# onesamblack/distributed-torch-horovod-gcp

Hardware: NVIDIA H100
Metric: images/sec (whole job, device-timed, max over ranks) ResNet-50 synthetic ImageNet training (higher is better)
Workload: dtype bf16

## Files before the change

### distributed_torch_horovod_gcp_b200/csrc/elementwise.cu

```cuda
#include <cuda_bf16.h>
#include <cuda_runtime.h>
#include <stdint.h>
#include <stdio.h>

namespace {

constexpr int THREADS = 256;

__device__ __forceinline__ void unpack8(const uint4& x, float* f) {
  const uint32_t w[4] = {x.x, x.y, x.z, x.w};
#pragma unroll
  for (int t = 0; t < 4; ++t) {
    f[2 * t] = __uint_as_float(w[t] << 16);
    f[2 * t + 1] = __uint_as_float(w[t] & 0xffff0000u);
  }
}
__device__ __forceinline__ uint4 pack8(const float* v) {
  uint32_t w[4];
#pragma unroll
  for (int t = 0; t < 4; ++t) {
    __nv_bfloat162 h = __floats2bfloat162_rn(v[2 * t], v[2 * t + 1]);
    w[t] = *reinterpret_cast<uint32_t*>(&h);
  }
  return make_uint4(w[0], w[1], w[2], w[3]);
}
__device__ __forceinline__ uint4 ldg_stream(const uint4* p) {
  uint4 v;
  asm volatile("ld.global.nc.L1::no_allocate.v4.u32 {%0,%1,%2,%3}, [%4];"
               : "=r"(v.x), "=r"(v.y), "=r"(v.z), "=r"(v.w)
               : "l"(p));
  return v;
}

constexpr int RED_MAX_BLOCKS = 256;
constexpr int RED_MAX_COLS = 2 * 2048;
__device__ float g_red_slots[RED_MAX_BLOCKS * RED_MAX_COLS];
__device__ unsigned int g_red_done;

template <int NACC, int NT>
__device__ __forceinline__ void block_reduce_to_global(float (&acc)[NACC][8], int V, float* const* outs) {
  __shared__ float sm[NT][8 + 1];
  __shared__ bool last;
  const int tid = threadIdx.x;
  const int groups = NT / V;
  const int C = V * 8;
  float* slot = g_red_slots + (size_t)blockIdx.x * (NACC * C);
#pragma unroll
  for (int q = 0; q < NACC; ++q) {
    __syncthreads();
#pragma unroll
    for (int j = 0; j < 8; ++j) sm[tid][j] = acc[q][j];
    __syncthreads();
    for (int item = tid; item < C; item += NT) {
      const int g0 = item >> 3, j = item & 7;
      float s = 0.f;
      for (int g = 0; g < groups; ++g) s += sm[g0 + g * V][j];
      slot[q * C + item] = s;
    }
  }
  __threadfence();
  __syncthreads();
  if (tid == 0) last = atomicAdd(&g_red_done, 1u) == gridDim.x - 1;
  __syncthreads();
  if (!last) return;
  __threadfence();
  for (int item = tid; item < NACC * C; item += NT) {
    float s = 0.f;
    for (unsigned b = 0; b < gridDim.x; ++b) s += __ldcg(g_red_slots + (size_t)b * (NACC * C) + item);
    outs[item / C][item % C] += s;
  }
  if (tid == 0) g_red_done = 0u;
}

constexpr int RTHREADS = 1024;

__device__ __forceinline__ uint4 ld_or_zero(const uint4* p, long long i, long long n) {
  return i < n ? ldg_stream(p + i) : make_uint4(0, 0, 0, 0);
}

__global__ void __launch_bounds__(RTHREADS, 1) bn_stats_kernel(const uint4* __restrict__ x, float* sum,
                                                               float* sumsq, long long nvec, int V) {
  constexpr int U = 8;
  float acc[2][8];
#pragma unroll
  for (int j = 0; j < 8; ++j) acc[0][j] = acc[1][j] = 0.f;
  const long long stride = (long long)gridDim.x * RTHREADS;
  for (long long i = (long long)blockIdx.x * RTHREADS + threadIdx.x; i < nvec; i += U * stride) {
    uint4 raw[U];
#pragma unroll
    for (int u = 0; u < U; ++u) raw[u] = ld_or_zero(x, i + u * stride, nvec);
#pragma unroll
    for (int u = 0; u < U; ++u) {
      float f[8];
      unpack8(raw[u], f);
#pragma unroll
      for (int j = 0; j < 8; ++j) {
        acc[0][j] += f[j];
        acc[1][j] = fmaf(f[j], f[j], acc[1][j]);
      }
    }
  }
  float* outs[2] = {sum, sumsq};
  block_reduce_to_global<2, RTHREADS>(acc, V, outs);
}

__device__ __forceinline__ float ld_param(const void* p, int c, int bf16) {
  return bf16 ? __bfloat162float(reinterpret_cast<const __nv_bfloat16*>(p)[c])
              : reinterpret_cast<const float*>(p)[c];
}
__device__ __forceinline__ void st_param(void* p, int c, int bf16, float v) {
  if (bf16) reinterpret_cast<__nv_bfloat16*>(p)[c] = __float2bfloat16_rn(v);
  else reinterpret_cast<float*>(p)[c] = v;
}

__global__ void bn_finalize_kernel(float* sum, float* sumsq, const void* gamma,
                                   const void* beta, float* mean, float* invstd, float* a, float* b,
                                   void* running_mean, void* running_var, float count, float eps,
                                   float momentum, int C, int pbf16, int rezero = 0,
                                   long long* num_batches_tracked = nullptr) {
  const int c = blockIdx.x * blockDim.x + threadIdx.x;
  if (c == 0 && num_batches_tracked != nullptr) *num_batches_tracked += 1;
  if (c >= C) return;
  const float m = sum[c] / count;
  const float var = fmaxf(sumsq[c] / count - m * m, 0.f);
  if (rezero) {
    sum[c] = 0.f;
    sumsq[c] = 0.f;
  }
  const float is = rsqrtf(var + eps);
  mean[c] = m;
  invstd[c] = is;
  const float g = gamma ? ld_param(gamma, c, pbf16) : 1.f;
  a[c] = g * is;
  b[c] = (beta ? ld_param(beta, c, pbf16) : 0.f) - m * g * is;
  if (running_mean) {
    const float unbiased = var * (count / fmaxf(count - 1.f, 1.f));
    st_param(running_mean, c, pbf16, (1.f - momentum) * ld_param(running_mean, c, pbf16) + momentum * m);
    st_param(running_var, c, pbf16,
             (1.f - momentum) * ld_param(running_var, c, pbf16) + momentum * unbiased);
  }
}

__global__ void __launch_bounds__(THREADS, 4) bn_apply_kernel(const uint4* __restrict__ x,
                                                              const uint4* __restrict__ res, uint4* y,
                                                              const float* __restrict__ a,
                                                              const float* __restrict__ b, long long nvec,
                                                              int V, int relu, uint8_t* __restrict__ mask) {
  constexpr int U = 4;
  const long long stride = (long long)gridDim.x * THREADS;
  const long long i0 = (long long)blockIdx.x * THREADS + threadIdx.x;
  if (i0 >= nvec) return;
  const int cg = (int)(i0 % V);
  float av[8], bv[8];
#pragma unroll
  for (int j = 0; j < 8; ++j) {
    av[j] = a[cg * 8 + j];
    bv[j] = b[cg * 8 + j];
  }
  for (long long i = i0; i < nvec; i += U * stride) {
    uint4 rx[U], rr[U];
#pragma unroll
    for (int u = 0; u < U; ++u) rx[u] = ld_or_zero(x, i + u * stride, nvec);
    if (res) {
#pragma unroll
      for (int u = 0; u < U; ++u) rr[u] = ld_or_zero(res, i + u * stride, nvec);
    }
#pragma unroll
    for (int u = 0; u < U; ++u) {
      if (i + u * stride >= nvec) break;
      float f[8];
      unpack8(rx[u], f);
#pragma unroll
      for (int j = 0; j < 8; ++j) f[j] = fmaf(f[j], av[j], bv[j]);
      if (res) {
        float r[8];
        unpack8(rr[u], r);
#pragma unroll
        for (int j = 0; j < 8; ++j) f[j] += r[j];
      }
      if (relu) {
        if (mask) {
          uint32_t m = 0;
#pragma unroll
          for (int j = 0; j < 8; ++j) m |= (f[j] > 0.f ? 1u : 0u) << j;
          mask[i + u * stride] = (uint8_t)m;
        }
#pragma unroll
        for (int j = 0; j < 8; ++j) f[j] = fmaxf(f[j], 0.f);
      }
      y[i + u * stride] = pack8(f);
    }
  }
}

__global__ void __launch_bounds__(RTHREADS, 1) bn_bwd_reduce_kernel(
    const uint4* __restrict__ dy, const uint4* __restrict__ x, const uint8_t* __restrict__ mask,
    const float* __restrict__ mean, float* sum_dy, float* sum_dy_xc, long long nvec, int V, int relu) {
  constexpr int U = 2;
  float acc[2][8];
#pragma unroll
  for (int j = 0; j < 8; ++j) acc[0][j] = acc[1][j] = 0.f;
  const long long stride = (long long)gridDim.x * RTHREADS;
  const long long i0 = (long long)blockIdx.x * RTHREADS + threadIdx.x;
  float mv[8];
  {
    const int cg = (int)(i0 % V);
#pragma unroll
    for (int j = 0; j < 8; ++j) mv[j] = mean[cg * 8 + j];
  }
  for (long long i = i0; i < nvec; i += U * stride) {
    uint4 rg[U], rx[U];
    uint32_t rm[U];
#pragma unroll
    for (int u = 0; u < U; ++u) {
      rg[u] = ld_or_zero(dy, i + u * stride, nvec);
      rx[u] = ld_or_zero(x, i + u * stride, nvec);
      rm[u] = (relu && i + u * stride < nvec) ? (uint32_t)__ldg(mask + i + u * stride) : 0xffu;
    }
#pragma unroll
    for (int u = 0; u < U; ++u) {
      float g[8], xv[8];
      unpack8(rg[u], g);
      unpack8(rx[u], xv);
#pragma unroll
      for (int j = 0; j < 8; ++j) g[j] = ((rm[u] >> j) & 1u) ? g[j] : 0.f;
#pragma unroll
      for (int j = 0; j < 8; ++j) {
        acc[0][j] += g[j];
        acc[1][j] = fmaf(g[j], xv[j] - mv[j], acc[1][j]);
      }
    }
  }
  float* outs[2] = {sum_dy, sum_dy_xc};
  block_reduce_to_global<2, RTHREADS>(acc, V, outs);
}

__global__ void __launch_bounds__(THREADS, 4) bn_bwd_apply_kernel(
    const uint4* __restrict__ dy, const uint4* __restrict__ x, const uint8_t* __restrict__ mask, uint4* dx,
    uint4* dres, const float* __restrict__ mean, const float* __restrict__ invstd,
    const float* __restrict__ scale_a, const float* __restrict__ sum_dy,
    const float* __restrict__ sum_dy_xhat, float inv_count, long long nvec, int V, int relu,
    void* dgamma, void* dbeta, int pbf16) {
  constexpr int U = 2;
  const long long stride = (long long)gridDim.x * THREADS;
  const long long i0 = (long long)blockIdx.x * THREADS + threadIdx.x;
  if (blockIdx.x == 0 && dgamma != nullptr) {
    for (int c = threadIdx.x; c < V * 8; c += THREADS) {
      st_param(dbeta, c, pbf16, sum_dy[c]);
      st_param(dgamma, c, pbf16, sum_dy_xhat[c] * invstd[c]);
    }
  }
  if (i0 >= nvec) return;
  const int cg = (int)(i0 % V);
  float mv[8], iv[8], k1[8], k2[8], sc[8];
#pragma unroll
  for (int j = 0; j < 8; ++j) {
    const int c = cg * 8 + j;
    mv[j] = mean[c];
    iv[j] = invstd[c];
    sc[j] = scale_a[c];
    k1[j] = sum_dy[c] * inv_count;
    k2[j] = sum_dy_xhat[c] * iv[j] * inv_count;
  }
  for (long long i = i0; i < nvec; i += U * stride) {
    uint4 rg[U], rx[U];
    uint32_t rm[U];
#pragma unroll
    for (int u = 0; u < U; ++u) {
      rg[u] = ld_or_zero(dy, i + u * stride, nvec);
      rx[u] = ld_or_zero(x, i + u * stride, nvec);
      rm[u] = (relu && i + u * stride < nvec) ? (uint32_t)__ldg(mask + i + u * stride) : 0xffu;
    }
#pragma unroll
    for (int u = 0; u < U; ++u) {
      if (i + u * stride >= nvec) break;
      float g[8], xv[8], o[8];
      unpack8(rg[u], g);
      unpack8(rx[u], xv);
#pragma unroll
      for (int j = 0; j < 8; ++j) g[j] = ((rm[u] >> j) & 1u) ? g[j] : 0.f;
#pragma unroll
      for (int j = 0; j < 8; ++j) {
        const float xhat = (xv[j] - mv[j]) * iv[j];
        o[j] = sc[j] * (g[j] - k1[j] - xhat * k2[j]);
      }
      dx[i + u * stride] = pack8(o);
      if (dres) dres[i + u * stride] = pack8(g);
    }
  }
}

constexpr int LN_WARPS = 16;

template <int VPL>
__global__ void __launch_bounds__(LN_WARPS * 32) ln_fwd_kernel(const uint4* __restrict__ x, uint4* __restrict__ y,
                                                               const void* gamma, const void* beta,
                                                               float* __restrict__ mean, float* __restrict__ rstd,
                                                               long long rows, float eps, int pbf16) {
  constexpr int C = 256 * VPL;
  const int lane = threadIdx.x & 31;
  const long long warp = (long long)blockIdx.x * LN_WARPS + (threadIdx.x >> 5);
  const long long nwarps = (long long)gridDim.x * LN_WARPS;
  float g[VPL][8], b[VPL][8];
#pragma unroll
  for (int v = 0; v < VPL; ++v)
#pragma unroll
    for (int j = 0; j < 8; ++j) {
      const int c = (v * 32 + lane) * 8 + j;
      g[v][j] = ld_param(gamma, c, pbf16);
      b[v][j] = ld_param(beta, c, pbf16);
    }
  for (long long r = warp; r < rows; r += nwarps) {
    const uint4* xr = x + r * (C / 8);
    float f[VPL][8];
    float s = 0.f;
#pragma unroll
    for (int v = 0; v < VPL; ++v) {
      unpack8(ldg_stream(xr + v * 32 + lane), f[v]);
#pragma unroll
      for (int j = 0; j < 8; ++j) s += f[v][j];
    }
#pragma unroll
    for (int o = 16; o > 0; o >>= 1) s += __shfl_xor_sync(0xffffffffu, s, o);
    const float m = s * (1.f / C);
    float q = 0.f;
#pragma unroll
    for (int v = 0; v < VPL; ++v)
#pragma unroll
      for (int j = 0; j < 8; ++j) {
        const float d = f[v][j] - m;
        q = fmaf(d, d, q);
      }
#pragma unroll
    for (int o = 16; o > 0; o >>= 1) q += __shfl_xor_sync(0xffffffffu, q, o);
    const float rs = rsqrtf(q * (1.f / C) + eps);
    if (lane == 0) {
      mean[r] = m;
      rstd[r] = rs;
    }
    uint4* yr = y + r * (C / 8);
#pragma unroll
    for (int v = 0; v < VPL; ++v) {
      float o[8];
#pragma unroll
      for (int j = 0; j < 8; ++j) o[j] = fmaf((f[v][j] - m) * rs, g[v][j], b[v][j]);
      yr[v * 32 + lane] = pack8(o);
    }
  }
}

template <int VPL>
__global__ void __launch_bounds__(LN_WARPS * 32) ln_bwd_kernel(const uint4* __restrict__ dy,
                                                               const uint4* __restrict__ x, uint4* __restrict__ dx,
                                                               const void* gamma, const float* __restrict__ mean,
                                                               const float* __restrict__ rstd, float* sums,
                                                               long long rows, int pbf16) {
  constexpr int C = 256 * VPL;
  extern __shared__ float red[];
  const int lane = threadIdx.x & 31, wib = threadIdx.x >> 5;
  const long long warp = (long long)blockIdx.x * LN_WARPS + wib;
  const long long nwarps = (long long)gridDim.x * LN_WARPS;
  float g[VPL][8], dg[VPL][8], db[VPL][8];
#pragma unroll
  for (int v = 0; v < VPL; ++v)
#pragma unroll
    for (int j = 0; j < 8; ++j) {
      g[v][j] = ld_param(gamma, (v * 32 + lane) * 8 + j, pbf16);
      dg[v][j] = db[v][j] = 0.f;
    }
  for (long long r = warp; r < rows; r += nwarps) {
    const float m = mean[r], rs = rstd[r];
// ... 202 lines not shown
  }
  const int vec_per_row = row_elems / 8;
  for (int i = threadIdx.x; i < 7 * vec_per_row; i += THREADS) {
    const int r = i / vec_per_row, v = i % vec_per_row;
    const int ih = oh * 2 - 3 + r;
    uint4 val = make_uint4(0, 0, 0, 0);
    if (ih >= 0 && ih < H)
      val = reinterpret_cast<const uint4*>(x + ((size_t)n * H + ih) * row_elems)[v];
    __nv_bfloat16* d = rows + r * pitch + 9 + v * 8;
    const __nv_bfloat16* sv = reinterpret_cast<const __nv_bfloat16*>(&val);
#pragma unroll
    for (int e = 0; e < 8; ++e) d[e] = sv[e];
  }
  __syncthreads();
  constexpr int UPR = STEM_KP / 8;
  uint4* dst = out + ((size_t)n * OH + oh) * OW * UPR;
  const uint32_t* rows32 = reinterpret_cast<const uint32_t*>(rows);
  const int pitch32 = pitch / 2;
  for (int i = threadIdx.x; i < OW * UPR; i += THREADS) {
    const int ow = i / UPR, u = i % UPR;
    const int kh = u / 3, part = u % 3;
    const uint32_t* src = rows32 + kh * pitch32 + ow * 3 + part * 4;
    dst[i] = make_uint4(src[0], src[1], src[2], src[3]);
  }
}


__global__ void __launch_bounds__(THREADS) avgpool_fwd_kernel(const uint4* __restrict__ x, uint4* __restrict__ y,
                                                              int HW, int V, long long total, float inv) {
  for (long long i = (long long)blockIdx.x * THREADS + threadIdx.x; i < total; i += (long long)gridDim.x * THREADS) {
    const long long n = i / V;
    const int v = (int)(i % V);
    const uint4* src = x + n * HW * V + v;
    float acc[8];
#pragma unroll
    for (int j = 0; j < 8; ++j) acc[j] = 0.f;
    for (int h = 0; h < HW; ++h) {
      float f[8];
      unpack8(src[(long long)h * V], f);
#pragma unroll
      for (int j = 0; j < 8; ++j) acc[j] += f[j];
    }
#pragma unroll
    for (int j = 0; j < 8; ++j) acc[j] *= inv;
    y[i] = pack8(acc);
  }
}
__global__ void __launch_bounds__(THREADS) avgpool_bwd_kernel(const uint4* __restrict__ dy, uint4* __restrict__ dx,
                                                              int HW, int V, long long total, float inv) {
  for (long long i = (long long)blockIdx.x * THREADS + threadIdx.x; i < total; i += (long long)gridDim.x * THREADS) {
    const long long n = i / ((long long)HW * V);
    const int v = (int)(i % V);
    float f[8];
    unpack8(dy[n * V + v], f);
#pragma unroll
    for (int j = 0; j < 8; ++j) f[j] *= inv;
    dx[i] = pack8(f);
  }
}

thread_local char g_err[256];
int fail(const char* what, cudaError_t e) {
  snprintf(g_err, sizeof(g_err), "%s: %s", what, cudaGetErrorString(e));
  return -1;
}

int g_sms = 0;
int reduce_grid() {
  if (g_sms == 0) {
    int dev = 0;
    cudaGetDevice(&dev);
    cudaDeviceGetAttribute(&g_sms, cudaDevAttrMultiProcessorCount, dev);
    if (g_sms <= 0) g_sms = 132;
    if (g_sms > RED_MAX_BLOCKS) g_sms = RED_MAX_BLOCKS;
  }
  return g_sms;
}

int grid_for(long long nvec, int V) {
  long long blocks = (nvec + THREADS * 8 - 1) / (THREADS * 8);
  if (blocks > (long long)reduce_grid() * 6) blocks = (long long)reduce_grid() * 6;
  if (blocks < 1) blocks = 1;
  return (int)blocks;
}

template <bool OUT_BF16>
__global__ void cast_acc_zero_kernel(float* __restrict__ src, void* __restrict__ dst, long long n4,
                                     int accumulate, int zero_src) {
  const long long stride = (long long)gridDim.x * blockDim.x;
  for (long long i = (long long)blockIdx.x * blockDim.x + threadIdx.x; i < n4; i += stride) {
    float4 v = reinterpret_cast<float4*>(src)[i];
    if (zero_src) reinterpret_cast<float4*>(src)[i] = make_float4(0.f, 0.f, 0.f, 0.f);
    if (OUT_BF16) {
      uint2* d = reinterpret_cast<uint2*>(dst) + i;
      if (accumulate) {
        const uint2 o = *d;
        v.x += __uint_as_float(o.x << 16); v.y += __uint_as_float(o.x & 0xffff0000u);
        v.z += __uint_as_float(o.y << 16); v.w += __uint_as_float(o.y & 0xffff0000u);
      }
      __nv_bfloat162 lo = __floats2bfloat162_rn(v.x, v.y), hi = __floats2bfloat162_rn(v.z, v.w);
      *d = make_uint2(*reinterpret_cast<uint32_t*>(&lo), *reinterpret_cast<uint32_t*>(&hi));
    } else {
      float4* d = reinterpret_cast<float4*>(dst) + i;
      if (accumulate) { const float4 o = *d; v.x += o.x; v.y += o.y; v.z += o.z; v.w += o.w; }
      *d = v;
    }
  }
}

bool shape_ok(int C) {
  const int V = C / 8;
  return C % 8 == 0 && V >= 1 && V <= THREADS && (THREADS % V) == 0;
}

}

extern "C" {

const char* b200dp_ew_last_error() { return g_err; }

int b200dp_cast_acc_zero(void* src, void* dst, long long n, int out_bf16, int accumulate, int zero_src,
                         unsigned long long stream) {
  if (n % 4) {
    snprintf(g_err, sizeof(g_err), "cast_acc_zero: n must be a multiple of 4");
    return -1;
  }
  const long long n4 = n / 4;
  int grid = (int)((n4 + 255) / 256);
  if (grid > reduce_grid() * 8) grid = reduce_grid() * 8;
  if (grid < 1) grid = 1;
  cudaStream_t st = (cudaStream_t)(uintptr_t)stream;
  if (out_bf16) cast_acc_zero_kernel<true><<<grid, 256, 0, st>>>((float*)src, dst, n4, accumulate, zero_src);
  else cast_acc_zero_kernel<false><<<grid, 256, 0, st>>>((float*)src, dst, n4, accumulate, zero_src);
  cudaError_t e = cudaGetLastError();
  if (e != cudaSuccess) return fail("cast_acc_zero launch", e);
  return 0;
}

int b200dp_bn_supported(int C) { return shape_ok(C) ? 1 : 0; }

int b200dp_bn_fwd(const void* x, const void* res, void* y, const void* gamma, const void* beta,
                  float* stats, float* mean, float* invstd, float* a, float* b, void* running_mean,
                  void* running_var, long long M, int C, float eps, float momentum, int relu,
                  int param_bf16, int have_stats, void* relu_mask, void* num_batches_tracked,
                  unsigned long long stream) {
  if (!shape_ok(C)) {
    snprintf(g_err, sizeof(g_err), "unsupported channel count %d", C);
    return -1;
  }
  cudaStream_t st = (cudaStream_t)(uintptr_t)stream;
  const int V = C / 8;
  const long long nvec = M * V;
  cudaError_t e = cudaSuccess;
  const int grid = grid_for(nvec, V);
  if (!have_stats) {
    e = cudaMemsetAsync(stats, 0, sizeof(float) * 2 * C, st);
    if (e != cudaSuccess) return fail("memset", e);
    bn_stats_kernel<<<reduce_grid(), RTHREADS, 0, st>>>((const uint4*)x, stats, stats + C, nvec, V);
  }
  bn_finalize_kernel<<<(C + 127) / 128, 128, 0, st>>>(stats, stats + C, gamma, beta, mean, invstd, a, b,
                                                      running_mean, running_var, (float)M, eps, momentum, C,
                                                      param_bf16, have_stats == 2 ? 1 : 0,
                                                      (long long*)num_batches_tracked);
  bn_apply_kernel<<<grid, THREADS, 0, st>>>((const uint4*)x, (const uint4*)res, (uint4*)y, a, b, nvec, V,
                                            relu, (uint8_t*)relu_mask);
  e = cudaGetLastError();
  if (e != cudaSuccess) return fail("bn_fwd launch", e);
  return 0;
}

int b200dp_bn_stats(const void* x, float* stats, long long M, int C, unsigned long long stream) {
  if (!shape_ok(C)) return -1;
  cudaStream_t st = (cudaStream_t)(uintptr_t)stream;
  cudaError_t e = cudaMemsetAsync(stats, 0, sizeof(float) * 2 * C, st);
  if (e != cudaSuccess) return fail("memset", e);
  bn_stats_kernel<<<reduce_grid(), RTHREADS, 0, st>>>((const uint4*)x, stats, stats + C, (long long)M * (C / 8),
                                                      C / 8);
  e = cudaGetLastError();
  if (e != cudaSuccess) return fail("bn_stats launch", e);
  return 0;
}

int b200dp_bn_fwd_sync(const void* x, const void* res, void* y, const void* gamma, const void* beta,
                       const float* stats, float* mean, float* invstd, float* a, float* b, void* running_mean,
                       void* running_var, long long M_local, double count, int C, float eps, float momentum,
                       int relu, int param_bf16, void* relu_mask, unsigned long long stream) {
  if (!shape_ok(C)) return -1;
  cudaStream_t st = (cudaStream_t)(uintptr_t)stream;
  const int V = C / 8;
  const long long nvec = M_local * V;
  bn_finalize_kernel<<<(C + 127) / 128, 128, 0, st>>>(const_cast<float*>(stats), const_cast<float*>(stats) + C, gamma,
                                                      beta, mean, invstd, a, b, running_mean, running_var,
                                                      (float)count, eps, momentum, C, param_bf16);
  bn_apply_kernel<<<grid_for(nvec, V), THREADS, 0, st>>>((const uint4*)x, (const uint4*)res, (uint4*)y, a, b, nvec,
                                                         V, relu, (uint8_t*)relu_mask);
  cudaError_t e = cudaGetLastError();
  if (e != cudaSuccess) return fail("bn_fwd_sync launch", e);
  return 0;
}

int b200dp_bn_bwd_reduce(const void* dy, const void* x, const void* relu_mask, const float* mean, float* sums,
                         long long M, int C, int relu, unsigned long long stream) {
  if (!shape_ok(C)) return -1;
  cudaStream_t st = (cudaStream_t)(uintptr_t)stream;
  cudaError_t e = cudaMemsetAsync(sums, 0, sizeof(float) * 2 * C, st);
  if (e != cudaSuccess) return fail("memset", e);
  bn_bwd_reduce_kernel<<<reduce_grid(), RTHREADS, 0, st>>>((const uint4*)dy, (const uint4*)x,
                                                           (const uint8_t*)relu_mask, mean, sums, sums + C,
                                                           (long long)M * (C / 8), C / 8, relu);
  e = cudaGetLastError();
  if (e != cudaSuccess) return fail("bn_bwd_reduce launch", e);
  return 0;
}

int b200dp_bn_bwd_apply(const void* dy, const void* x, const void* relu_mask, void* dx, void* dres,
                        const float* scale_a, const float* mean, const float* invstd, const float* sums,
                        double count, long long M, int C, int relu, unsigned long long stream) {
  if (!shape_ok(C)) return -1;
  const int V = C / 8;
  const long long nvec = M * V;
  bn_bwd_apply_kernel<<<grid_for(nvec, V), THREADS, 0, (cudaStream_t)(uintptr_t)stream>>>(
      (const uint4*)dy, (const uint4*)x, (const uint8_t*)relu_mask, (uint4*)dx, (uint4*)dres, mean, invstd, scale_a,
      sums, sums + C, (float)(1.0 / count), nvec, V, relu, nullptr, nullptr, 0);
  cudaError_t e = cudaGetLastError();
  if (e != cudaSuccess) return fail("bn_bwd_apply launch", e);
  return 0;
}

int b200dp_bn_apply(const void* x, const void* res, void* y, const float* a, const float* b, long long M,
                    int C, int relu, unsigned long long stream) {
  if (!shape_ok(C)) return -1;
  const int V = C / 8;
  const long long nvec = M * V;
  bn_apply_kernel<<<grid_for(nvec, V), THREADS, 0, (cudaStream_t)(uintptr_t)stream>>>(
      (const uint4*)x, (const uint4*)res, (uint4*)y, a, b, nvec, V, relu, nullptr);
  cudaError_t e = cudaGetLastError();
  if (e != cudaSuccess) return fail("bn_apply launch", e);
  return 0;
}

int b200dp_bn_bwd(const void* dy, const void* x, const void* relu_mask, void* dx, void* dres, const float* scale_a,
                  const float* mean, const float* invstd, float* sums, void* dgamma, void* dbeta,
                  int param_bf16, long long M, int C, int relu, unsigned long long stream) {
  if (!shape_ok(C)) return -1;
  cudaStream_t st = (cudaStream_t)(uintptr_t)stream;
  const int V = C / 8;
  const long long nvec = M * V;
  cudaError_t e = cudaMemsetAsync(sums, 0, sizeof(float) * 2 * C, st);
  if (e != cudaSuccess) return fail("memset", e);
  const int grid = grid_for(nvec, V);
  bn_bwd_reduce_kernel<<<reduce_grid(), RTHREADS, 0, st>>>((const uint4*)dy, (const uint4*)x,
                                                           (const uint8_t*)relu_mask, mean, sums, sums + C,
                                                           nvec, V, relu);
  bn_bwd_apply_kernel<<<grid, THREADS, 0, st>>>((const uint4*)dy, (const uint4*)x, (const uint8_t*)relu_mask,
                                                (uint4*)dx, (uint4*)dres, mean, invstd, scale_a, sums,
                                                sums + C, 1.0f / (float)M, nvec, V, relu, dgamma, dbeta,
                                                param_bf16);
  e = cudaGetLastError();
  if (e != cudaSuccess) return fail("bn_bwd launch", e);
  return 0;
}

int b200dp_maxpool_fwd(const void* x, void* y, void* idx, int N, int H, int W, int C,
                       unsigned long long stream) {
  if (C % 8) return -1;
  const int OH = (H + 2 - 3) / 2 + 1, OW = (W + 2 - 3) / 2 + 1, V = C / 8;
  const long long total = (long long)N * OH * OW * V;
  int grid = (int)((total + THREADS - 1) / THREADS);
  if (grid > reduce_grid() * 16) grid = reduce_grid() * 16;
  maxpool_fwd_kernel<<<grid, THREADS, 0, (cudaStream_t)(uintptr_t)stream>>>((const uint4*)x, (uint4*)y,
                                                                             (uint2*)idx, N, H, W, OH, OW, V);
  cudaError_t e = cudaGetLastError();
  if (e != cudaSuccess) return fail("maxpool_fwd launch", e);
  return 0;
}

int b200dp_maxpool_bwd(const void* dy, const void* idx, void* dx, int N, int H, int W, int C,
                       unsigned long long stream) {
  if (C % 8) return -1;
  const int OH = (H + 2 - 3) / 2 + 1, OW = (W + 2 - 3) / 2 + 1, V = C / 8;
  if (H % 2 == 0 && W % 2 == 0) {
    const long long patches = (long long)N * (H / 2) * (W / 2) * V;
    int pgrid = (int)((patches + THREADS - 1) / THREADS);
    if (pgrid > reduce_grid() * 16) pgrid = reduce_grid() * 16;
    maxpool_bwd_patch_kernel<<<pgrid, THREADS, 0, (cudaStream_t)(uintptr_t)stream>>>(
        (const uint4*)dy, (const uint2*)idx, (uint4*)dx, N, H, W, OH, OW, V);
    cudaError_t pe = cudaGetLastError();
    if (pe != cudaSuccess) return fail("maxpool_bwd launch", pe);
    return 0;
  }
  const long long total = (long long)N * H * W * V;
  int grid = (int)((total + THREADS - 1) / THREADS);
  if (grid > reduce_grid() * 16) grid = reduce_grid() * 16;
  maxpool_bwd_kernel<<<grid, THREADS, 0, (cudaStream_t)(uintptr_t)stream>>>((const uint4*)dy, (const uint2*)idx,
                                                                             (uint4*)dx, N, H, W, OH, OW, V);
  cudaError_t e = cudaGetLastError();
  if (e != cudaSuccess) return fail("maxpool_bwd launch", e);
  return 0;
}

int b200dp_avgpool_fwd(const void* x, void* y, long long N, int HW, int C, unsigned long long stream) {
  if (C % 8) return -1;
  const int V = C / 8;
  const long long total = N * V;
  int grid = (int)((total + THREADS - 1) / THREADS);
  if (grid > reduce_grid() * 8) grid = reduce_grid() * 8;
  avgpool_fwd_kernel<<<grid, THREADS, 0, (cudaStream_t)(uintptr_t)stream>>>((const uint4*)x, (uint4*)y, HW, V, total,
                                                                             1.0f / (float)HW);
  cudaError_t e = cudaGetLastError();
  if (e != cudaSuccess) return fail("avgpool_fwd launch", e);
  return 0;
}

int b200dp_avgpool_bwd(const void* dy, void* dx, long long N, int HW, int C, unsigned long long stream) {
  if (C % 8) return -1;
  const int V = C / 8;
  const long long total = N * HW * V;
  int grid = (int)((total + THREADS - 1) / THREADS);
  if (grid > reduce_grid() * 8) grid = reduce_grid() * 8;
  avgpool_bwd_kernel<<<grid, THREADS, 0, (cudaStream_t)(uintptr_t)stream>>>((const uint4*)dy, (uint4*)dx, HW, V, total,
                                                                             1.0f / (float)HW);
  cudaError_t e = cudaGetLastError();
  if (e != cudaSuccess) return fail("avgpool_bwd launch", e);
  return 0;
}

int b200dp_stem_im2col(const void* x, void* out, int N, int H, int W, unsigned long long stream) {
  if ((W % 8) || (H % 2)) return -1;
  const int OH = H / 2, OW = W / 2;
  const size_t smem = (size_t)7 * ((9 + W * 3 + 15 + 7) & ~7) * sizeof(__nv_bfloat16);
  stem_im2col_kernel<<<N * OH, THREADS, smem, (cudaStream_t)(uintptr_t)stream>>>(
      (const __nv_bfloat16*)x, (uint4*)out, H, W, OH, OW);
  cudaError_t e = cudaGetLastError();
  if (e != cudaSuccess) return fail("stem_im2col launch", e);
  return 0;
}

int b200dp_ln_supported(int C) { return (C % 256 == 0 && C / 256 >= 1 && C / 256 <= 4) ? 1 : 0; }

int b200dp_ln_fwd(const void* x, void* y, const void* gamma, const void* beta, float* mean, float* rstd,
                  long long rows, int C, float eps, int param_bf16, unsigned long long stream) {
// ... 43 lines not shown
```

### distributed_torch_horovod_gcp_b200/ops/bn.py

```python
from __future__ import annotations

import ctypes
import os
from typing import Optional

import torch
import torch.nn.functional as F

from . import counters
from . import gemm as _gemm
from . import grad_sink

_lib = None
_USE_GEMM_1X1 = os.environ.get("B200DP_CONV1X1_GEMM", "1") == "1"


def register(lib, have):
    global _lib
    if not hasattr(lib, "b200dp_bn_fwd"):
        return
    _lib = lib
    vp, i, f, ll, u64 = ctypes.c_void_p, ctypes.c_int, ctypes.c_float, ctypes.c_longlong, ctypes.c_uint64
    lib.b200dp_bn_fwd.argtypes = [vp, vp, vp, vp, vp, vp, vp, vp, vp, vp, vp, vp, ll, i, f, f, i, i, i, vp, vp, u64]
    lib.b200dp_bn_apply.argtypes = [vp, vp, vp, vp, vp, ll, i, i, u64]
    lib.b200dp_bn_bwd.argtypes = [vp, vp, vp, vp, vp, vp, vp, vp, vp, vp, vp, i, ll, i, i, u64]
    lib.b200dp_bn_supported.argtypes = [i]
    if hasattr(lib, "b200dp_bn_fwd_sync"):
        d = ctypes.c_double
        lib.b200dp_bn_stats.argtypes = [vp, vp, ll, i, u64]
        lib.b200dp_bn_fwd_sync.argtypes = [vp] * 12 + [ll, d, i, f, f, i, i, vp, u64]
        lib.b200dp_bn_bwd_reduce.argtypes = [vp, vp, vp, vp, vp, ll, i, i, u64]
        lib.b200dp_bn_bwd_apply.argtypes = [vp] * 9 + [d, ll, i, i, u64]
    lib.b200dp_ew_last_error.restype = ctypes.c_char_p
    have["bn_act"] = True
    have["conv_bn_act"] = True
    if hasattr(lib, "b200dp_stem_im2col"):
        lib.b200dp_stem_im2col.argtypes = [vp, vp, i, i, i, u64]
        have["stem_conv"] = True
    if hasattr(lib, "b200dp_avgpool_fwd"):
        lib.b200dp_avgpool_fwd.argtypes = [vp, vp, ctypes.c_longlong, i, i, u64]
        lib.b200dp_avgpool_bwd.argtypes = [vp, vp, ctypes.c_longlong, i, i, u64]
        have["global_avg_pool"] = True
    if hasattr(lib, "b200dp_maxpool_fwd"):
        lib.b200dp_maxpool_fwd.argtypes = [vp, vp, vp, i, i, i, i, u64]
        lib.b200dp_maxpool_bwd.argtypes = [vp, vp, vp, i, i, i, i, u64]
        have["max_pool_3x3_s2"] = True


def _ck(rc):
    if rc != 0:
        raise RuntimeError("elementwise kernel: " + (_lib.b200dp_ew_last_error() or b"").decode())


def _nhwc_ok(x: torch.Tensor) -> bool:
    return x.dim() == 4 and x.dtype == torch.bfloat16 and \
        x.is_contiguous(memory_format=torch.channels_last) and x.data_ptr() % 16 == 0


def bn_supported(x: torch.Tensor, C: int) -> bool:
    return _lib is not None and _nhwc_ok(x) and bool(_lib.b200dp_bn_supported(C))


def _cl(t: torch.Tensor) -> torch.Tensor:
    return t if t.is_contiguous(memory_format=torch.channels_last) else t.contiguous(memory_format=torch.channels_last)


def bn_forward(x, bn: torch.nn.BatchNorm2d, residual, relu: bool, stats_in=None, grads=(True, True)):
    N, C, H, W = x.shape
    M = N * H * W
    dev = x.device
    gamma, beta = bn.weight, bn.bias
    nbt = bn.num_batches_tracked if (bn.track_running_stats and bn.num_batches_tracked is not None
                                     and bn.num_batches_tracked.is_cuda) else None
    mom = bn.momentum if bn.momentum is not None else 0.1
    y = torch.empty_like(x, memory_format=torch.channels_last)
    ws = torch.empty(6 * C, dtype=torch.float32, device=dev)
    stats, mean, invstd, a, b = ws[:2 * C], ws[2 * C:3 * C], ws[3 * C:4 * C], ws[4 * C:5 * C], ws[5 * C:]
    if stats_in is not None:
        stats = stats_in
    pbf16 = int(gamma.dtype == torch.bfloat16)
    mask = torch.empty(M * (C // 8), dtype=torch.uint8, device=dev) if relu else None
    st = torch.cuda.current_stream(dev).cuda_stream
    _ck(_lib.b200dp_bn_fwd(x.data_ptr(), residual.data_ptr() if residual is not None else None,
                           y.data_ptr(), gamma.data_ptr(), beta.data_ptr(), stats.data_ptr(),
                           mean.data_ptr(), invstd.data_ptr(), a.data_ptr(), b.data_ptr(),
                           bn.running_mean.data_ptr() if bn.running_mean is not None else None,
                           bn.running_var.data_ptr() if bn.running_var is not None else None,
                           M, C, float(bn.eps), float(mom), int(relu), pbf16,
                           2 if stats_in is not None else 0,
                           mask.data_ptr() if mask is not None else None,
                           nbt.data_ptr() if nbt is not None else None, st))
    counters.bump("bn_fwd", 2 if stats_in is not None else 3)
    if grads[0]:
        grad_sink.note_forward(gamma)
    if grads[1]:
        grad_sink.note_forward(beta)
    return y, mask, (mean, invstd, a)


def bn_backward(dy, bn: torch.nn.BatchNorm2d, x, mask, ws, write_dres: bool = False):
    mean, invstd, a = ws
    N, C, H, W = x.shape
    M = N * H * W
    dx = torch.empty_like(x, memory_format=torch.channels_last)
    dres = torch.empty_like(x, memory_format=torch.channels_last) if write_dres else None
    sums = torch.empty(2 * C, dtype=torch.float32, device=x.device)
    gamma, beta = bn.weight, bn.bias
    gd, ga, gdone = grad_sink.begin(gamma)
    bd, ba, bdone = grad_sink.begin(beta)
    direct = gd is not None and bd is not None and not ga and not ba
    if direct:
        dg_ptr, db_ptr = gd.data_ptr(), bd.data_ptr()
    else:
        dgb = torch.empty(2 * C, dtype=gamma.dtype, device=x.device)
        dg_ptr, db_ptr = dgb.data_ptr(), dgb.data_ptr() + C * dgb.element_size()
    st = torch.cuda.current_stream(x.device).cuda_stream
    _ck(_lib.b200dp_bn_bwd(dy.data_ptr(), x.data_ptr(), mask.data_ptr() if mask is not None else None,
                           dx.data_ptr(), dres.data_ptr() if dres is not None else None,
                           a.data_ptr(), mean.data_ptr(), invstd.data_ptr(), sums.data_ptr(),
                           dg_ptr, db_ptr,
                           int(gamma.dtype == torch.bfloat16), M, C, int(mask is not None), st))
    counters.bump("bn_bwd", 2)
    if direct:
        gdone()
        bdone()
        return dx, None, None, dres
    return dx, dgb[:C], dgb[C:], dres


class _BNActFn(torch.autograd.Function):

    @staticmethod
    def forward(ctx, x, gamma, beta, residual, relu, stats_in, bn):
        y, mask, ws = bn_forward(x, bn, residual, relu, stats_in, ctx.needs_input_grad[1:3])
# ... 199 lines not shown
```

Measured before the change: 5708.

## Launch BN kernels with programmatic dependent launch and drop stats memsets

The BatchNorm kernels are now launched with cudaLaunchKernelEx and the programmatic stream serialization attribute, so each kernel's prologue can overlap the tail of the previous one. The cross-block final reduction now overwrites its outputs instead of accumulating, which removes the cudaMemsetAsync before each stats and backward reduce. The last-block slot summation is restructured to use register batching or shared-memory staging. The backward apply kernel issues its first loads before griddepcontrol.wait. This trims launch gaps and memset launches across the many small BN kernels per step, at the cost of more complex sync whose correctness depends on the wait placement.

```diff
diff --git a/distributed_torch_horovod_gcp_b200/csrc/elementwise.cu b/distributed_torch_horovod_gcp_b200/csrc/elementwise.cu
--- a/distributed_torch_horovod_gcp_b200/csrc/elementwise.cu
+++ b/distributed_torch_horovod_gcp_b200/csrc/elementwise.cu
@@ -2,6 +2,7 @@
 #include <cuda_runtime.h>
 #include <stdint.h>
 #include <stdio.h>
+#include <stdlib.h>
 
 namespace {
 
@@ -32,10 +33,65 @@
   return v;
 }
 
+__device__ __forceinline__ void pdl_wait() { asm volatile("griddepcontrol.wait;" ::: "memory"); }
+__device__ __forceinline__ void pdl_launch_dependents() { asm volatile("griddepcontrol.launch_dependents;" ::: "memory"); }
+
 constexpr int RED_MAX_BLOCKS = 256;
 constexpr int RED_MAX_COLS = 2 * 2048;
 __device__ float g_red_slots[RED_MAX_BLOCKS * RED_MAX_COLS];
 __device__ unsigned int g_red_done;
+
+template <int J, int NT>
+__device__ __forceinline__ void sum_slots_regs(int C, float* const* outs) {
+  constexpr int R = 32 / J;
+  const int NI = J * NT;
+  const unsigned G = gridDim.x;
+  float s[J];
+#pragma unroll
+  for (int j = 0; j < J; ++j) s[j] = 0.f;
+  for (unsigned b0 = 0; b0 < G; b0 += R) {
+    float v[J][R];
+#pragma unroll
+    for (int j = 0; j < J; ++j)
+#pragma unroll
+      for (int r = 0; r < R; ++r)
+        v[j][r] = b0 + r < G ? __ldcg(g_red_slots + (size_t)(b0 + r) * NI + threadIdx.x + j * NT) : 0.f;
+#pragma unroll
+    for (int j = 0; j < J; ++j)
+#pragma unroll
+      for (int r = 0; r < R; ++r)
+        if (b0 + r < G) s[j] += v[j][r];
+  }
+#pragma unroll
+  for (int j = 0; j < J; ++j) {
+    const int item = threadIdx.x + j * NT;
+    outs[item / C][item % C] = 0.f + s[j];
+  }
+}
+
+template <int NT>
+__device__ __forceinline__ void sum_slots_staged(int NI, int C, float* stage, float* const* outs) {
+  const int tid = threadIdx.x;
+  const unsigned G = gridDim.x;
+  const unsigned SB = (NT * 8) / NI;
+  float s = 0.f;
+  for (unsigned b0 = 0; b0 < G; b0 += SB) {
+    const int n = (int)min(SB, G - b0) * NI;
+    const float* src = g_red_slots + (size_t)b0 * NI;
+    float v[8];
+#pragma unroll
+    for (int r = 0; r < 8; ++r)
+      if (tid + r * NT < n) v[r] = __ldcg(src + tid + r * NT);
+    __syncthreads();
+#pragma unroll
+    for (int r = 0; r < 8; ++r)
+      if (tid + r * NT < n) stage[tid + r * NT] = v[r];
+    __syncthreads();
+    if (tid < NI)
+      for (int k = tid; k < n; k += NI) s += stage[k];
+  }
+  if (tid < NI) outs[tid / C][tid % C] = 0.f + s;
+}
 
 template <int NACC, int NT>
 __device__ __forceinline__ void block_reduce_to_global(float (&acc)[NACC][8], int V, float* const* outs) {
@@ -64,11 +120,11 @@
   __syncthreads();
   if (!last) return;
   __threadfence();
-  for (int item = tid; item < NACC * C; item += NT) {
-    float s = 0.f;
-    for (unsigned b = 0; b < gridDim.x; ++b) s += __ldcg(g_red_slots + (size_t)b * (NACC * C) + item);
-    outs[item / C][item % C] += s;
-  }
+  const int NI = NACC * C;
+  if (NI < NT) sum_slots_staged<NT>(NI, C, &sm[0][0], outs);
+  else if (NI == NT) sum_slots_regs<1, NT>(C, outs);
+  else if (NI == 2 * NT) sum_slots_regs<2, NT>(C, outs);
+  else sum_slots_regs<4, NT>(C, outs);
   if (tid == 0) g_red_done = 0u;
 }
 
@@ -81,6 +137,8 @@
 __global__ void __launch_bounds__(RTHREADS, 1) bn_stats_kernel(const uint4* __restrict__ x, float* sum,
                                                                float* sumsq, long long nvec, int V) {
   constexpr int U = 8;
+  pdl_wait();
+  pdl_launch_dependents();
   float acc[2][8];
 #pragma unroll
   for (int j = 0; j < 8; ++j) acc[0][j] = acc[1][j] = 0.f;
@@ -116,9 +174,11 @@
 __global__ void bn_finalize_kernel(float* sum, float* sumsq, const void* gamma,
                                    const void* beta, float* mean, float* invstd, float* a, float* b,
                                    void* running_mean, void* running_var, float count, float eps,
-                                   float momentum, int C, int pbf16, int rezero = 0,
-                                   long long* num_batches_tracked = nullptr) {
+                                   float momentum, int C, int pbf16, int rezero,
+                                   long long* num_batches_tracked) {
   const int c = blockIdx.x * blockDim.x + threadIdx.x;
+  pdl_wait();
+  pdl_launch_dependents();
   if (c == 0 && num_batches_tracked != nullptr) *num_batches_tracked += 1;
   if (c >= C) return;
   const float m = sum[c] / count;
@@ -149,6 +209,8 @@
   constexpr int U = 4;
   const long long stride = (long long)gridDim.x * THREADS;
   const long long i0 = (long long)blockIdx.x * THREADS + threadIdx.x;
+  pdl_wait();
+  pdl_launch_dependents();
   if (i0 >= nvec) return;
   const int cg = (int)(i0 % V);
   float av[8], bv[8];
@@ -197,6 +259,8 @@
     const uint4* __restrict__ dy, const uint4* __restrict__ x, const uint8_t* __restrict__ mask,
     const float* __restrict__ mean, float* sum_dy, float* sum_dy_xc, long long nvec, int V, int relu) {
   constexpr int U = 2;
+  pdl_wait();
+  pdl_launch_dependents();
   float acc[2][8];
 #pragma unroll
   for (int j = 0; j < 8; ++j) acc[0][j] = acc[1][j] = 0.f;
@@ -244,6 +308,19 @@
   constexpr int U = 2;
   const long long stride = (long long)gridDim.x * THREADS;
   const long long i0 = (long long)blockIdx.x * THREADS + threadIdx.x;
+  uint4 rg[U], rx[U];
+  uint32_t rm[U];
+  auto load = [&](long long i) {
+#pragma unroll
+    for (int u = 0; u < U; ++u) {
+      rg[u] = ld_or_zero(dy, i + u * stride, nvec);
+      rx[u] = ld_or_zero(x, i + u * stride, nvec);
+      rm[u] = (relu && i + u * stride < nvec) ? (uint32_t)__ldg(mask + i + u * stride) : 0xffu;
+    }
+  };
+  if (i0 < nvec) load(i0);
+  pdl_wait();
+  pdl_launch_dependents();
   if (blockIdx.x == 0 && dgamma != nullptr) {
     for (int c = threadIdx.x; c < V * 8; c += THREADS) {
       st_param(dbeta, c, pbf16, sum_dy[c]);
@@ -262,15 +339,7 @@
     k1[j] = sum_dy[c] * inv_count;
     k2[j] = sum_dy_xhat[c] * iv[j] * inv_count;
   }
-  for (long long i = i0; i < nvec; i += U * stride) {
-    uint4 rg[U], rx[U];
-    uint32_t rm[U];
-#pragma unroll
-    for (int u = 0; u < U; ++u) {
-      rg[u] = ld_or_zero(dy, i + u * stride, nvec);
-      rx[u] = ld_or_zero(x, i + u * stride, nvec);
-      rm[u] = (relu && i + u * stride < nvec) ? (uint32_t)__ldg(mask + i + u * stride) : 0xffu;
-    }
+  auto apply = [&](long long i) {
 #pragma unroll
     for (int u = 0; u < U; ++u) {
       if (i + u * stride >= nvec) break;
@@ -287,6 +356,11 @@
       dx[i + u * stride] = pack8(o);
       if (dres) dres[i + u * stride] = pack8(g);
     }
+  };
+  apply(i0);
+  for (long long i = i0 + U * stride; i < nvec; i += U * stride) {
+    load(i);
+    apply(i);
   }
 }
 
@@ -655,6 +729,29 @@
   if (blocks > (long long)reduce_grid() * 6) blocks = (long long)reduce_grid() * 6;
   if (blocks < 1) blocks = 1;
   return (int)blocks;
+}
+
+int g_bn_pdl = -1;
+bool bn_pdl() {
+  if (g_bn_pdl < 0) {
+    const char* e = getenv("B200DP_BN_PDL");
+    g_bn_pdl = (e != nullptr && e[0] == '0') ? 0 : 1;
+  }
+  return g_bn_pdl != 0;
+}
+
+template <typename... KArgs, typename... Args>
+cudaError_t bn_launch(void (*kern)(KArgs...), int grid, int block, cudaStream_t st, Args... args) {
+  cudaLaunchAttribute attr[1];
+  attr[0].id = cudaLaunchAttributeProgrammaticStreamSerialization;
+  attr[0].val.programmaticStreamSerializationAllowed = 1;
+  cudaLaunchConfig_t cfg = {};
+  cfg.gridDim = dim3(grid);
+  cfg.blockDim = dim3(block);
+  cfg.stream = st;
+  cfg.attrs = attr;
+  cfg.numAttrs = bn_pdl() ? 1 : 0;
+  return cudaLaunchKernelEx(&cfg, kern, static_cast<KArgs>(args)...);
 }
 
 template <bool OUT_BF16>
@@ -712,6 +809,12 @@
 
 int b200dp_bn_supported(int C) { return shape_ok(C) ? 1 : 0; }
 
+int b200dp_bn_set_pdl(int on) {
+  const int prev = bn_pdl() ? 1 : 0;
+  if (on >= 0) g_bn_pdl = on ? 1 : 0;
+  return prev;
+}
+
 int b200dp_bn_fwd(const void* x, const void* res, void* y, const void* gamma, const void* beta,
                   float* stats, float* mean, float* invstd, float* a, float* b, void* running_mean,
                   void* running_var, long long M, int C, float eps, float momentum, int relu,
@@ -725,31 +828,23 @@
   const int V = C / 8;
   const long long nvec = M * V;
   cudaError_t e = cudaSuccess;
-  const int grid = grid_for(nvec, V);
-  if (!have_stats) {
-    e = cudaMemsetAsync(stats, 0, sizeof(float) * 2 * C, st);
-    if (e != cudaSuccess) return fail("memset", e);
-    bn_stats_kernel<<<reduce_grid(), RTHREADS, 0, st>>>((const uint4*)x, stats, stats + C, nvec, V);
-  }
-  bn_finalize_kernel<<<(C + 127) / 128, 128, 0, st>>>(stats, stats + C, gamma, beta, mean, invstd, a, b,
-                                                      running_mean, running_var, (float)M, eps, momentum, C,
-                                                      param_bf16, have_stats == 2 ? 1 : 0,
-                                                      (long long*)num_batches_tracked);
-  bn_apply_kernel<<<grid, THREADS, 0, st>>>((const uint4*)x, (const uint4*)res, (uint4*)y, a, b, nvec, V,
-                                            relu, (uint8_t*)relu_mask);
-  e = cudaGetLastError();
+  if (!have_stats)
+    e = bn_launch(bn_stats_kernel, reduce_grid(), RTHREADS, st, (const uint4*)x, stats, stats + C, nvec, V);
+  if (e == cudaSuccess)
+    e = bn_launch(bn_finalize_kernel, (C + 127) / 128, 128, st, stats, stats + C, gamma, beta, mean, invstd, a, b,
+                  running_mean, running_var, (float)M, eps, momentum, C, param_bf16, have_stats == 2 ? 1 : 0,
+                  (long long*)num_batches_tracked);
+  if (e == cudaSuccess)
+    e = bn_launch(bn_apply_kernel, grid_for(nvec, V), THREADS, st, (const uint4*)x, (const uint4*)res, (uint4*)y,
+                  a, b, nvec, V, relu, (uint8_t*)relu_mask);
   if (e != cudaSuccess) return fail("bn_fwd launch", e);
   return 0;
 }
 
 int b200dp_bn_stats(const void* x, float* stats, long long M, int C, unsigned long long stream) {
   if (!shape_ok(C)) return -1;
-  cudaStream_t st = (cudaStream_t)(uintptr_t)stream;
-  cudaError_t e = cudaMemsetAsync(stats, 0, sizeof(float) * 2 * C, st);
-  if (e != cudaSuccess) return fail("memset", e);
-  bn_stats_kernel<<<reduce_grid(), RTHREADS, 0, st>>>((const uint4*)x, stats, stats + C, (long long)M * (C / 8),
-                                                      C / 8);
-  e = cudaGetLastError();
+  const cudaError_t e = bn_launch(bn_stats_kernel, reduce_grid(), RTHREADS, (cudaStream_t)(uintptr_t)stream,
+                                  (const uint4*)x, stats, stats + C, (long long)M * (C / 8), C / 8);
   if (e != cudaSuccess) return fail("bn_stats launch", e);
   return 0;
 }
@@ -762,12 +857,12 @@
   cudaStream_t st = (cudaStream_t)(uintptr_t)stream;
   const int V = C / 8;
   const long long nvec = M_local * V;
-  bn_finalize_kernel<<<(C + 127) / 128, 128, 0, st>>>(const_cast<float*>(stats), const_cast<float*>(stats) + C, gamma,
-                                                      beta, mean, invstd, a, b, running_mean, running_var,
-                                                      (float)count, eps, momentum, C, param_bf16);
-  bn_apply_kernel<<<grid_for(nvec, V), THREADS, 0, st>>>((const uint4*)x, (const uint4*)res, (uint4*)y, a, b, nvec,
-                                                         V, relu, (uint8_t*)relu_mask);
-  cudaError_t e = cudaGetLastError();
+  cudaError_t e = bn_launch(bn_finalize_kernel, (C + 127) / 128, 128, st, const_cast<float*>(stats),
+                            const_cast<float*>(stats) + C, gamma, beta, mean, invstd, a, b, running_mean, running_var,
+                            (float)count, eps, momentum, C, param_bf16, 0, (long long*)nullptr);
+  if (e == cudaSuccess)
+    e = bn_launch(bn_apply_kernel, grid_for(nvec, V), THREADS, st, (const uint4*)x, (const uint4*)res, (uint4*)y,
+                  a, b, nvec, V, relu, (uint8_t*)relu_mask);
   if (e != cudaSuccess) return fail("bn_fwd_sync launch", e);
   return 0;
 }
@@ -775,13 +870,9 @@
 int b200dp_bn_bwd_reduce(const void* dy, const void* x, const void* relu_mask, const float* mean, float* sums,
                          long long M, int C, int relu, unsigned long long stream) {
   if (!shape_ok(C)) return -1;
-  cudaStream_t st = (cudaStream_t)(uintptr_t)stream;
-  cudaError_t e = cudaMemsetAsync(sums, 0, sizeof(float) * 2 * C, st);
-  if (e != cudaSuccess) return fail("memset", e);
-  bn_bwd_reduce_kernel<<<reduce_grid(), RTHREADS, 0, st>>>((const uint4*)dy, (const uint4*)x,
-                                                           (const uint8_t*)relu_mask, mean, sums, sums + C,
-                                                           (long long)M * (C / 8), C / 8, relu);
-  e = cudaGetLastError();
+  const cudaError_t e = bn_launch(bn_bwd_reduce_kernel, reduce_grid(), RTHREADS, (cudaStream_t)(uintptr_t)stream,
+                                  (const uint4*)dy, (const uint4*)x, (const uint8_t*)relu_mask, mean, sums, sums + C,
+                                  (long long)M * (C / 8), C / 8, relu);
   if (e != cudaSuccess) return fail("bn_bwd_reduce launch", e);
   return 0;
 }
@@ -792,10 +883,10 @@
   if (!shape_ok(C)) return -1;
   const int V = C / 8;
   const long long nvec = M * V;
-  bn_bwd_apply_kernel<<<grid_for(nvec, V), THREADS, 0, (cudaStream_t)(uintptr_t)stream>>>(
-      (const uint4*)dy, (const uint4*)x, (const uint8_t*)relu_mask, (uint4*)dx, (uint4*)dres, mean, invstd, scale_a,
-      sums, sums + C, (float)(1.0 / count), nvec, V, relu, nullptr, nullptr, 0);
-  cudaError_t e = cudaGetLastError();
+  const cudaError_t e = bn_launch(bn_bwd_apply_kernel, grid_for(nvec, V), THREADS, (cudaStream_t)(uintptr_t)stream,
+                                  (const uint4*)dy, (const uint4*)x, (const uint8_t*)relu_mask, (uint4*)dx,
+                                  (uint4*)dres, mean, invstd, scale_a, sums, sums + C, (float)(1.0 / count), nvec, V,
+                                  relu, (void*)nullptr, (void*)nullptr, 0);
   if (e != cudaSuccess) return fail("bn_bwd_apply launch", e);
   return 0;
 }
@@ -805,9 +896,9 @@
   if (!shape_ok(C)) return -1;
   const int V = C / 8;
   const long long nvec = M * V;
-  bn_apply_kernel<<<grid_for(nvec, V), THREADS, 0, (cudaStream_t)(uintptr_t)stream>>>(
-      (const uint4*)x, (const uint4*)res, (uint4*)y, a, b, nvec, V, relu, nullptr);
-  cudaError_t e = cudaGetLastError();
+  const cudaError_t e = bn_launch(bn_apply_kernel, grid_for(nvec, V), THREADS, (cudaStream_t)(uintptr_t)stream,
+                                  (const uint4*)x, (const uint4*)res, (uint4*)y, a, b, nvec, V, relu,
+                                  (uint8_t*)nullptr);
   if (e != cudaSuccess) return fail("bn_apply launch", e);
   return 0;
 }
@@ -819,17 +910,12 @@
   cudaStream_t st = (cudaStream_t)(uintptr_t)stream;
   const int V = C / 8;
   const long long nvec = M * V;
-  cudaError_t e = cudaMemsetAsync(sums, 0, sizeof(float) * 2 * C, st);
-  if (e != cudaSuccess) return fail("memset", e);
-  const int grid = grid_for(nvec, V);
-  bn_bwd_reduce_kernel<<<reduce_grid(), RTHREADS, 0, st>>>((const uint4*)dy, (const uint4*)x,
-                                                           (const uint8_t*)relu_mask, mean, sums, sums + C,
-                                                           nvec, V, relu);
-  bn_bwd_apply_kernel<<<grid, THREADS, 0, st>>>((const uint4*)dy, (const uint4*)x, (const uint8_t*)relu_mask,
-                                                (uint4*)dx, (uint4*)dres, mean, invstd, scale_a, sums,
-                                                sums + C, 1.0f / (float)M, nvec, V, relu, dgamma, dbeta,
-                                                param_bf16);
-  e = cudaGetLastError();
+  cudaError_t e = bn_launch(bn_bwd_reduce_kernel, reduce_grid(), RTHREADS, st, (const uint4*)dy, (const uint4*)x,
+                            (const uint8_t*)relu_mask, mean, sums, sums + C, nvec, V, relu);
+  if (e == cudaSuccess)
+    e = bn_launch(bn_bwd_apply_kernel, grid_for(nvec, V), THREADS, st, (const uint4*)dy, (const uint4*)x,
+                  (const uint8_t*)relu_mask, (uint4*)dx, (uint4*)dres, mean, invstd, scale_a, sums, sums + C,
+                  1.0f / (float)M, nvec, V, relu, dgamma, dbeta, param_bf16);
   if (e != cudaSuccess) return fail("bn_bwd launch", e);
   return 0;
 }
diff --git a/distributed_torch_horovod_gcp_b200/ops/bn.py b/distributed_torch_horovod_gcp_b200/ops/bn.py
--- a/distributed_torch_horovod_gcp_b200/ops/bn.py
+++ b/distributed_torch_horovod_gcp_b200/ops/bn.py
@@ -25,6 +25,7 @@
     lib.b200dp_bn_apply.argtypes = [vp, vp, vp, vp, vp, ll, i, i, u64]
     lib.b200dp_bn_bwd.argtypes = [vp, vp, vp, vp, vp, vp, vp, vp, vp, vp, vp, i, ll, i, i, u64]
     lib.b200dp_bn_supported.argtypes = [i]
+    lib.b200dp_bn_set_pdl.argtypes = [i]
     if hasattr(lib, "b200dp_bn_fwd_sync"):
         d = ctypes.c_double
         lib.b200dp_bn_stats.argtypes = [vp, vp, ll, i, u64]
@@ -50,6 +51,10 @@
 def _ck(rc):
     if rc != 0:
         raise RuntimeError("elementwise kernel: " + (_lib.b200dp_ew_last_error() or b"").decode())
+
+
+def set_pdl(on: bool) -> bool:
+    return bool(_lib.b200dp_bn_set_pdl(int(on)))
 
 
 def _nhwc_ok(x: torch.Tensor) -> bool:
```

Result: no change. 5740, median of 6 (+0.6%).
